# ginevracoal/robustBNNs

Measured on AMD Instinct MI355X. Metric: attack-samples/sec (test_pts x posterior_samples x PGD_iters), higher is better.
Workload: dtype f32 (full-width operands as three f16 pieces: 6 exact f16 MFMA product terms per fp32 product, f32 accumulate)

## Files before the change

include/robustbnns_hip.h:

```cpp
#ifndef ROBUSTBNNS_HIP_H
#define ROBUSTBNNS_HIP_H

#include <stddef.h>
#include <stdint.h>

#ifdef __cplusplus
extern "C" {
#endif

#define RBNN_ABI_VERSION 10
#define RBNN_CPAD 16

typedef enum rbnn_status {
    RBNN_OK = 0,
    RBNN_ERR_NULL = -1,
    RBNN_ERR_SHAPE = -2,
    RBNN_ERR_UNSUPPORTED = -3,
    RBNN_ERR_LAUNCH = -4,
    RBNN_ERR_ALIGN = -5
} rbnn_status;

typedef enum rbnn_activation { RBNN_ACT_RELU = 0, RBNN_ACT_LEAKY = 1, RBNN_ACT_SIGM = 2, RBNN_ACT_TANH = 3 } rbnn_activation;
typedef enum rbnn_arch { RBNN_ARCH_FC = 0, RBNN_ARCH_FC2 = 1 } rbnn_arch;

// ... 49 lines not shown
int rbnn_reduce_samples(const float *P, int32_t n_samples, int32_t n_points, int32_t n_classes,
                        float scale, float *out, int32_t ldo, void *stream);

int rbnn_loss_dlogits(int32_t mode, const float *P, const float *Psum, int32_t ldp, const float *G_up,
                      const int32_t *labels, int32_t n_samples, float inv_S, int32_t n_points,
                      int32_t n_classes, float *dZ, void *stream);

int rbnn_fc_input_grad(const rbnn_posterior *net, const int32_t *sample_idx, int32_t n_samples,
                       int32_t n_points, int32_t chunk, const rbnn_workspace *ws,
                       int32_t *n_slabs_out, void *stream);

int rbnn_sum_slabs(const float *slabs, int32_t n_slabs, int32_t n_points, int32_t d_pad, float scale,
                   float *out, int32_t ldo, void *stream);

int rbnn_sum_slabs_norms(const float *slabs, int32_t n_slabs, int32_t n_points, int32_t d_pad, int32_t in_features, float scale,
                         float *out, int32_t ldo, float *linf, float *l2, void *stream);

int rbnn_pgd_alpha(const float *X0, int32_t ldx, int32_t n_points, int32_t in_features,
                   float *alpha, void *stream);

int rbnn_attack_step(float *X, const float *X0, int32_t ldx, const float *G, int32_t n_slabs,
                     size_t slab_stride, int32_t ldg, const float *alpha, float alpha_scalar,
                     float eps, int32_t project, int32_t n_points, int32_t in_features, void *stream);

int rbnn_eval_metrics(const float *out_orig, const float *out_adv, int32_t ldp, const int32_t *labels,
                      int32_t n_points, int32_t n_classes, int32_t *counts, float *rob, void *stream);

int rbnn_pack_rows4(const float *W, int64_t rows, int32_t cols, float *out, void *stream);

typedef struct rbnn_dev_scale {
    uint32_t absmax_bits;
    int32_t  exp;
    float    scale;
    float    inv_scale;
} rbnn_dev_scale;

int rbnn_input_scales(const float *X, int64_t rows, int32_t cols, int32_t ld, float floor_abs, float mul, float add,
                      float cap, rbnn_dev_scale *out, void *stream);

typedef struct rbnn_conv_posterior {
    int32_t activation;
    int32_t hidden;
    int32_t n_classes;
    int32_t n_stored;
    int32_t in_channels;
    int32_t in_width;
// ... 577 lines not shown
```

robustbnns_amd/_hip.py:

```python
import ctypes as C
import os

import torch

from . import _header
from ._header import HipError

_HERE = os.path.dirname(os.path.abspath(__file__))
LIB_PATH = os.path.join(_HERE, "csrc", "librbnn_hip.so")
HEADER_PATH = os.path.join(os.path.dirname(_HERE), "include", "robustbnns_hip.h")

STRUCTS = {
    "Posterior": "rbnn_posterior", "Workspace": "rbnn_workspace", "WorkspaceSizes": "rbnn_workspace_sizes",
    "ConvPosterior": "rbnn_conv_posterior", "ConvWorkspace": "rbnn_conv_workspace", "ConvWorkspaceSizes": "rbnn_conv_workspace_sizes",
    "PieceImages": "rbnn_triple_images", "SplitImages": "rbnn_triple_images", "TripleImages": "rbnn_triple_images",
    "SplitWorkspace": "rbnn_split_workspace", "SplitWorkspaceSizes": "rbnn_split_workspace_sizes",
    "TripleWorkspace": "rbnn_triple_workspace", "TripleWorkspaceSizes": "rbnn_triple_workspace_sizes",
    "SviGuide": "rbnn_svi_guide", "SviFlatTensor": "rbnn_svi_flat_tensor", "SviTrainNet": "rbnn_svi_train_net", "SviTrainWs": "rbnn_svi_train_ws",
    "NnTrainNet": "rbnn_nn_train_net", "NnTrainWs": "rbnn_nn_train_ws",
    "ConvTrainNet": "rbnn_conv_train_net", "ConvTrainWs": "rbnn_conv_train_ws", "ConvTrainBytes": "rbnn_conv_train_bytes",
    "ConvSviTrainNet": "rbnn_conv_svi_train_net",
    "ConvEnsNet": "rbnn_conv_ens_net", "ConvEnsWs": "rbnn_conv_ens_ws", "ConvEnsBytes": "rbnn_conv_ens_bytes",
    "ConvSviLockstepNet": "rbnn_conv_svi_guides_net", "ConvSviLockstepWs": "rbnn_conv_svi_guides_ws", "ConvSviLockstepBytes": "rbnn_conv_svi_guides_bytes",
    "HmcChain": "rbnn_hmc_chain", "HmcLockstep": "rbnn_hmc_lockstep", "ConvHmcChainsNet": "rbnn_conv_hmc_chains_net", "SviLockstep": "rbnn_svi_multi", "SviLockstepAcc": "rbnn_svi_multi_acc",
# ... 120 lines not shown
        check(self.lib.rbnn_loss_dlogits(mode, ptr(P), ptr(Psum), ldp, ptr(G_up), ptr(labels), S, inv_S, N, Cn,
                                         ptr(dZ), stream_of(P)), "rbnn_loss_dlogits")

    def fc_input_grad(self, net, sidx, S, N, chunk, ws):
        w = self._ws(ws)
        n = C.c_int32(0)
        check(self.lib.rbnn_fc_input_grad(C.byref(net.descriptor()), ptr(sidx), S, N, chunk, C.byref(w), C.byref(n),
                                          stream_of(ws["dZ"])), "rbnn_fc_input_grad")
        return n.value

    def sum_slabs(self, slabs, K, N, Dp, scale, out):
        require_gpu(slabs, "slabs")
        check(self.lib.rbnn_sum_slabs(ptr(slabs), K, N, Dp, scale, ptr(out), out.stride(0), stream_of(slabs)), "rbnn_sum_slabs")

    def sum_slabs_norms(self, slabs, K, N, Dp, D, scale, out, linf, l2):
        require_gpu(slabs, "slabs")
        check(self.lib.rbnn_sum_slabs_norms(ptr(slabs), K, N, Dp, D, scale, ptr(out), out.stride(0), ptr(linf), ptr(l2),
                                            stream_of(slabs)), "rbnn_sum_slabs_norms")

    def pgd_alpha(self, X0, D, alpha):
        require_gpu(X0, "X0")
        check(self.lib.rbnn_pgd_alpha(ptr(X0), X0.stride(0), X0.shape[0], D, ptr(alpha), stream_of(X0)), "rbnn_pgd_alpha")

    def attack_step(self, X, X0, G, K, slab_stride, ldg, alpha, alpha_scalar, eps, project, D):
        require_gpu(X, "X")
        check(self.lib.rbnn_attack_step(ptr(X), ptr(X0), X.stride(0), ptr(G), K, slab_stride, ldg, ptr(alpha),
                                        alpha_scalar, eps, int(project), X.shape[0], D, stream_of(X)), "rbnn_attack_step")

    def eval_metrics(self, A, B, labels, Cn, counts, rob):
        require_gpu(A, "outputs")
        check(self.lib.rbnn_eval_metrics(ptr(A), ptr(B), A.stride(0), ptr(labels), A.shape[0], Cn, ptr(counts), ptr(rob),
                                         stream_of(A)), "rbnn_eval_metrics")

    def pack_rows4(self, W, out):
        require_gpu(W, "W")
        cols = W.shape[-1]
        check(self.lib.rbnn_pack_rows4(ptr(W), W.numel() // cols, cols, ptr(out), stream_of(W)), "rbnn_pack_rows4")

    def input_scales(self, X, cols, floor_abs, mul, add, cap, out):
        require_gpu(X, "X")
        check(self.lib.rbnn_input_scales(ptr(X), X.shape[0], cols, X.stride(0), floor_abs, mul, add, cap, ptr(out), stream_of(X)),
              "rbnn_input_scales")
        return out

    def _rows_image(self, name, src, cols, scale_exp, out, ld_dst, dev_scale):
        require_gpu(src, "src")
        ld_src = src.shape[-1]
        check(getattr(self.lib, name)(ptr(src), src.numel() // ld_src, cols, ld_src, scale_exp, ptr(dev_scale), ptr(out), ld_dst, stream_of(src)), name)
# ... 247 lines not shown
```

robustbnns_amd/csrc/rbnn_kernels.hip:

```cpp
#include "rbnn_common.hpp"
#include <stdlib.h>

namespace {

struct FwdArgs {
    const float* X;   long long x_sample_stride;  int ldx;  int N;
    const float* W;   long long w_sample_stride;  int ldw;  int KT;
    const float* b;
    const float* W2;  const float* b2;            int C;    int H;
    const int* sidx;  int S;   int NT;
    float* P;  uint32_t* mask;  float* dact;  float* hid;  int out_kind;
};

template <int ACT, int WH, int HTW, int WN, int NTW, bool LAYER2>
__global__ void __launch_bounds__(64 * WH * WN, (HTW * NTW > 16 ? 2 : (WH * WN) / 2)) fc_forward_kernel(const FwdArgs a) {
    constexpr int BH = WH * HTW * 16, BN = WN * NTW * 16;
    constexpr int TILE = (BH + BN) * 16;
    constexpr bool BITMASK = (ACT == RBNN_ACT_RELU || ACT == RBNN_ACT_LEAKY);
    constexpr int NW = WH * WN;
    static_assert(NW == 4 || NW == 8, "4 or 8 waves per block");
    static_assert(HTW % 2 == 0 && HTW <= 8, "a wave's h range is whole 32-bit mask words, at most 4");
    static_assert(WH * BN * 16 <= 2 * TILE, "the Z^T reduction scratch aliases the tile buffers");
    __shared__ __attribute__((aligned(16))) float lds[2 * TILE];
    float* const zred = lds;
// ... 468 lines not shown

__global__ void attack_step4_kernel(float* __restrict__ X, const float* __restrict__ X0, int ldx,
                                    const float* __restrict__ G, int K, long long slab_stride, int ldg,
                                    const float* __restrict__ alpha, float alpha_scalar, float eps, int project,
                                    int N, int D4) {
    const long long i = (long long)blockIdx.x * blockDim.x + threadIdx.x;
    if (i >= (long long)N * D4) return;
    const long long n = i / D4;
    const int d = 4 * (int)(i % D4);
    f32x4 g = *(const f32x4*)(G + n * ldg + d);
    for (int k = 1; k < K; ++k) g += *(const f32x4*)(G + k * slab_stride + n * ldg + d);
    const float step = alpha ? alpha[n] : alpha_scalar;
    const f32x4 x = *(const f32x4*)(X + n * ldx + d);
    f32x4 x0 = x, out;
    if (project) x0 = *(const f32x4*)(X0 + n * ldx + d);
#pragma unroll
    for (int r = 0; r < 4; ++r) {
        const float sgn = (g[r] > 0.f) ? 1.f : ((g[r] < 0.f) ? -1.f : 0.f);
        float pert = x[r] + step * sgn;
        if (project) pert = x0[r] + fminf(fmaxf(pert - x0[r], -eps), eps);
        out[r] = fminf(fmaxf(pert, 0.f), 1.f);
    }
    *(f32x4*)(X + n * ldx + d) = out;
}

__global__ void eval_metrics_kernel(const float* __restrict__ A, const float* __restrict__ B, int ldp,
                                    const int* __restrict__ labels, int N, int C, int* __restrict__ counts,
                                    float* __restrict__ rob) {
    const int n = blockIdx.x * blockDim.x + threadIdx.x;
    int ok_a = 0, ok_b = 0;
    if (n < N) {
        float ma = -INFINITY, mb = -INFINITY;
        int ia = 0, ib = 0;
        for (int c = 0; c < C; ++c) {
            const float a = A[(long long)n * ldp + c], b = B[(long long)n * ldp + c];
            if (a > ma) { ma = a; ia = c; }
            if (b > mb) { mb = b; ib = c; }
        }
        float da = 0.f, db = 0.f;
        for (int c = 0; c < C; ++c) { da += expf(A[(long long)n * ldp + c] - ma); db += expf(B[(long long)n * ldp + c] - mb); }
        float diff = 0.f;
        for (int c = 0; c < C; ++c)
            diff = fmaxf(diff, fabsf(expf(A[(long long)n * ldp + c] - ma) / da - expf(B[(long long)n * ldp + c] - mb) / db));
        rob[n] = 1.f - diff;
        ok_a = (ia == labels[n]);
        ok_b = (ib == labels[n]);
// ... 277 lines not shown
int rbnn_pgd_alpha(const float* X0, int32_t ldx, int32_t N, int32_t D, float* alpha, void* stream) {
    if (!X0 || !alpha) return RBNN_ERR_NULL;
    if (N < 1 || D < 1 || ldx < D) return RBNN_ERR_SHAPE;
    hipLaunchKernelGGL(pgd_alpha_kernel, dim3((N + 3) / 4), dim3(256), 0, (hipStream_t)stream, X0, ldx, N, D, alpha);
    return launch_status();
}

int rbnn_attack_step(float* X, const float* X0, int32_t ldx, const float* G, int32_t K, size_t slab_stride, int32_t ldg,
                     const float* alpha, float alpha_scalar, float eps, int32_t project, int32_t N, int32_t D, void* stream) {
    if (!X || !G || (project && !X0)) return RBNN_ERR_NULL;
    if (N < 1 || D < 1 || ldx < D || ldg < D || K < 1) return RBNN_ERR_SHAPE;
    if (!(D & 3) && !(ldx & 3) && !(ldg & 3) && !(slab_stride & 3) && aligned16(X) && aligned16(G) && (!project || aligned16(X0))) {
        const long long total4 = (long long)N * (D / 4);
        hipLaunchKernelGGL(attack_step4_kernel, dim3((unsigned)((total4 + 255) / 256)), dim3(256), 0, (hipStream_t)stream,
                           X, X0, ldx, G, K, (long long)slab_stride, ldg, alpha, alpha_scalar, eps, project, N, D / 4);
        return launch_status();
    }
    const long long total = (long long)N * D;
    hipLaunchKernelGGL(attack_step_kernel, dim3((unsigned)((total + 255) / 256)), dim3(256), 0, (hipStream_t)stream,
                       X, X0, ldx, G, K, (long long)slab_stride, ldg, alpha, alpha_scalar, eps, project, N, D);
    return launch_status();
}

int rbnn_eval_metrics(const float* out_orig, const float* out_adv, int32_t ldp, const int32_t* labels, int32_t N, int32_t C,
                      int32_t* counts, float* rob, void* stream) {
    if (!out_orig || !out_adv || !labels || !counts || !rob) return RBNN_ERR_NULL;
    if (N < 1 || C < 1 || ldp < C) return RBNN_ERR_SHAPE;
    if (hipMemsetAsync(counts, 0, 2 * sizeof(int32_t), (hipStream_t)stream) != hipSuccess) return RBNN_ERR_LAUNCH;
    hipLaunchKernelGGL(eval_metrics_kernel, dim3((N + 255) / 256), dim3(256), 0, (hipStream_t)stream,
                       out_orig, out_adv, ldp, labels, N, C, counts, rob);
    return launch_status();
}

int rbnn_pack_rows4(const float* W, int64_t rows, int32_t cols, float* out, void* stream) {
    if (!W || !out) return RBNN_ERR_NULL;
    if (rows < 4 || (rows & 3) || cols < 1) return RBNN_ERR_SHAPE;
    if (!aligned16(out)) return RBNN_ERR_ALIGN;
    const long long total = (rows / 4) * (long long)cols;
    hipLaunchKernelGGL(pack_rows4_kernel, dim3((unsigned)((total + 255) / 256)), dim3(256), 0, (hipStream_t)stream, W, (long long)(rows / 4), cols, out);
    return launch_status();
}

int rbnn_svi_materialize(const float* loc, const float* scale_raw, const float* eps, int64_t n_elem, int32_t S, float* out, void* stream) {
    if (!loc || !scale_raw || !eps || !out) return RBNN_ERR_NULL;
    if (n_elem < 1 || S < 1) return RBNN_ERR_SHAPE;
    const long long total = (long long)n_elem * S;
// ... 10 lines not shown
```

robustbnns_amd/csrc/rbnn_svi.hip:

```cpp
#include "rbnn_common.hpp"
#include <algorithm>

namespace {

struct DrawArgs {
    rbnn_posterior net;
    rbnn_triple_images tp;
    rbnn_svi_guide g;
    const unsigned long long* sample_keys;
    unsigned long long key;
    uint32_t draw_id;
    int S, has_tp, tiles_w1_d, tiles_wm_d, tiles_per_sample;
    int images_only;
    float w1_scale, wm_scale, w2_scale;
};

__device__ void draw_matrix_tile(const DrawArgs& a, const Rng& rng, int tensor, int s, int hb, int dt, const float* loc, const float* scl,
                                 int H0, int cols, float* W, int ldw, float* pack4, uint4* rows_img, int ld_rows, uint4* cols_img, int ld_cols,
                                 float img_scale, float (*tile)[68]) {
    const int H = a.net.hidden, t = threadIdx.x, d0 = 64 * dt;
#pragma unroll
    for (int i = 0; i < 2; ++i) {
        const int q = t + 256 * i, hl = q >> 4, dq = q & 15;
        const int h = 32 * hb + hl, c4 = (d0 >> 2) + dq;
        float w[4] = {0.f, 0.f, 0.f, 0.f};
        if (h < H0 && 4 * c4 < cols) draw_quad(rng, tensor, loc, scl, h, c4, cols, w);
        *(f32x4*)&tile[hl][4 * dq] = (f32x4){w[0], w[1], w[2], w[3]};
    }
    __syncthreads();
    if (W) {
#pragma unroll
        for (int i = 0; i < 2; ++i) {
            const int q = t + 256 * i, hl = q >> 4, dq = q & 15, d = d0 + 4 * dq;
            if (d < ldw) *(f32x4*)(W + ((long long)s * H + 32 * hb + hl) * ldw + d) = *(const f32x4*)&tile[hl][4 * dq];
        }
    }
    if (pack4) {
// ... 70 lines not shown
        const int lane = i & 63, li = lane & 15, lg = lane >> 4, k = (i >> 6) & 1, tl = i >> 7;
        _Float16 w[10][3];
#pragma unroll
        for (int c = 0; c < 10; ++c) pieces_of<3>((c < C) ? w2l[c * H + 16 * tl + li] * a.w2_scale : 0.f, w[c]);
        union { f16x8 v; uint4 u; } o;
        const _Float16 z = (_Float16)0.f;
        if (lg < 3) {
            const int piece = (k == 0) ? (lg == 2 ? 1 : 0) : (lg == 0 ? 1 : (lg == 1 ? 0 : 2));
#pragma unroll
            for (int j = 0; j < 8; ++j) o.v[j] = piece == 0 ? w[j][0] : (piece == 1 ? w[j][1] : w[j][2]);
        } else if (k == 0) {
            o.v[0] = w[8][0]; o.v[1] = w[9][0]; o.v[2] = w[8][0]; o.v[3] = w[9][0];
            o.v[4] = w[8][0]; o.v[5] = w[9][0]; o.v[6] = w[8][1]; o.v[7] = w[9][1];
        } else {
            o.v[0] = w[8][2]; o.v[1] = w[9][2]; o.v[2] = w[8][1]; o.v[3] = w[9][1];
            o.v[4] = z; o.v[5] = z; o.v[6] = z; o.v[7] = z;
        }
        gen[i] = o.u;
    }
}

__global__ void __launch_bounds__(256) svi_draw_kernel(const DrawArgs a) {
    extern __shared__ float dyn_lds[];
    const int s = blockIdx.x / a.tiles_per_sample, j = blockIdx.x % a.tiles_per_sample;
    const unsigned long long key = a.sample_keys ? a.sample_keys[s] : a.key;
    const Rng rng = {(uint32_t)key, (uint32_t)(key >> 32), a.sample_keys ? 0u : (uint32_t)s, a.draw_id};
    const int H = a.net.hidden;
    const int n_w1 = (H / 32) * a.tiles_w1_d, n_wm = (H / 32) * a.tiles_wm_d;
    float (*tile)[68] = (float (*)[68])dyn_lds;
    if (j < n_w1) {
        draw_matrix_tile(a, rng, T_W1, s, j / a.tiles_w1_d, j % a.tiles_w1_d, a.g.W1_loc, a.g.W1_scale, a.g.hidden, a.net.in_features,
                         a.images_only ? nullptr : const_cast<float*>(a.net.W1), a.net.in_stride, a.images_only ? nullptr : const_cast<float*>(a.net.W1_pack4),
                         a.has_tp ? (uint4*)const_cast<void*>(a.tp.W1_rows) : nullptr, a.tp.ld_rows,
                         a.has_tp ? (uint4*)const_cast<void*>(a.tp.W1_cols) : nullptr, a.tp.ld_cols, a.w1_scale, tile);
    } else if (j < n_w1 + n_wm) {
        const int jj = j - n_w1;
        draw_matrix_tile(a, rng, T_WM, s, jj / a.tiles_wm_d, jj % a.tiles_wm_d, a.g.Wm_loc, a.g.Wm_scale, a.g.hidden, a.g.hidden,
                         a.images_only ? nullptr : const_cast<float*>(a.net.Wm), H, a.images_only ? nullptr : const_cast<float*>(a.net.Wm_pack4),
                         a.has_tp ? (uint4*)const_cast<void*>(a.tp.Wm_rows) : nullptr, H,
                         a.has_tp ? (uint4*)const_cast<void*>(a.tp.Wm_cols) : nullptr, H, a.wm_scale, tile);
    } else {
        draw_small(a, rng, s, dyn_lds);
    }
}


struct FlatArgs {
// ... 69 lines not shown
    if (images_only && !tp) return RBNN_ERR_NULL;
    if (!g->W1_loc || !g->W1_scale || !g->b1_loc || !g->b1_scale || !g->W2_loc || !g->W2_scale || !g->b2_loc || !g->b2_scale) return RBNN_ERR_NULL;
    if (net->arch != RBNN_ARCH_FC && net->arch != RBNN_ARCH_FC2) return RBNN_ERR_UNSUPPORTED;
    const bool fc2 = net->arch == RBNN_ARCH_FC2;
    if (fc2 && (!net->Wm || !net->bm || !g->Wm_loc || !g->Wm_scale || !g->bm_loc || !g->bm_scale)) return RBNN_ERR_NULL;
    const int H = net->hidden, C = net->n_classes;
    if (n_samples < 1 || n_samples > net->n_stored || H < 32 || (H & 31) || g->hidden < 1 || g->hidden > H || C < 1 || C > 16) return RBNN_ERR_SHAPE;
    if (net->in_features < 1 || net->in_stride < net->in_features || (net->in_stride & 15)) return RBNN_ERR_SHAPE;
    DrawArgs a = {};
    a.net = *net; a.g = *g; a.sample_keys = (const unsigned long long*)sample_keys; a.key = key; a.draw_id = draw_id; a.S = n_samples;
    a.images_only = images_only;
    int extent = net->in_stride;
    if (tp) {
        if (!tp->W1_rows || !tp->W1_cols || !tp->W2_gen || (fc2 && (!tp->Wm_rows || !tp->Wm_cols))) return RBNN_ERR_NULL;
        if (tp->ld_rows < net->in_features || (tp->ld_rows & 31) || tp->ld_cols != net->in_stride || C > 10 || (H & 127)) return RBNN_ERR_SHAPE;
        if (tp->w1_exp < -100 || tp->w1_exp > 100 || tp->w2_exp < -100 || tp->w2_exp > 100 || tp->wm_exp < -100 || tp->wm_exp > 100) return RBNN_ERR_SHAPE;
        a.tp = *tp; a.has_tp = 1;
        a.w1_scale = ldexpf(1.f, tp->w1_exp); a.w2_scale = ldexpf(1.f, tp->w2_exp); a.wm_scale = ldexpf(1.f, tp->wm_exp);
        extent = std::max(extent, (int)tp->ld_rows);
    }
    a.tiles_w1_d = (extent + 63) / 64;
    a.tiles_wm_d = fc2 ? (H + 63) / 64 : 0;
    a.tiles_per_sample = (H / 32) * (a.tiles_w1_d + a.tiles_wm_d) + 1;
    const size_t lds = std::max((size_t)32 * 68 * sizeof(float), (size_t)C * H * sizeof(float));
    if (lds > SVI_DRAW_LDS_MAX) return RBNN_ERR_SHAPE;
    static unsigned long long attr = 0;
    if (lds > 64 * 1024 && !ensure_dynamic_lds((const void*)svi_draw_kernel, (int)SVI_DRAW_LDS_MAX, attr)) return RBNN_ERR_LAUNCH;
    hipLaunchKernelGGL(svi_draw_kernel, dim3((unsigned)((long long)n_samples * a.tiles_per_sample)), dim3(256), lds, (hipStream_t)stream, a);
    return launch_status();
}

int rbnn_svi_draw(const rbnn_posterior* net, const rbnn_triple_images* tp, const rbnn_svi_guide* g, int32_t n_samples,
                  const uint64_t* sample_keys, uint64_t key, uint32_t draw_id, void* stream) {
    return svi_draw_impl(net, tp, g, n_samples, sample_keys, key, draw_id, 0, stream);
}

int rbnn_svi_draw_images(const rbnn_posterior* net, const rbnn_triple_images* tp, const rbnn_svi_guide* g, int32_t n_samples,
                         const uint64_t* sample_keys, uint64_t key, uint32_t draw_id, void* stream) {
    return svi_draw_impl(net, tp, g, n_samples, sample_keys, key, draw_id, 1, stream);
}

}

#include "rbnn_svi_step.hpp"
#include "rbnn_conv_layout.hpp"

// ... 34 lines not shown
```

robustbnns_amd/csrc/rbnn_triple.hip:

```cpp
#include "rbnn_pieces.hpp"
#include <algorithm>
#include <cstdlib>

namespace {

#ifndef RBNN_X3_PAIR_NOP
#define RBNN_X3_PAIR_NOP 0
#endif
#if RBNN_X3_PAIR_NOP
#define RBNN_X3_PAIR_PAD "\n\ts_nop 1"
#else
#define RBNN_X3_PAIR_PAD ""
#endif
#define RBNN_X3_PAIR_BODY \
    "v_bfe_i32 %[me], %[mw], %[b0], 1\n\t" \
    "v_bfe_i32 %[mo], %[mw], %[b1], 1\n\t" \
    "v_bfi_b32 %[me], %[me], %[cp], %[cn]\n\t" \
    "v_bfi_b32 %[mo], %[mo], %[cp], %[cn]\n\t" \
    "v_fma_mixlo_f16 %[d0], %[ge], %[me], 0\n\t" \
    "v_fma_mixhi_f16 %[d0], %[go], %[mo], 0\n\t" \
    "v_fma_mix_f32 %[re], %[ge], %[me], -%[d0] op_sel_hi:[0,0,1]\n\t" \
    "v_fma_mix_f32 %[ro], %[go], %[mo], -%[d0] op_sel:[0,0,1] op_sel_hi:[0,0,1]\n\t" \
    "v_cvt_pk_f16_f32 %[d1], %[re], %[ro]\n\t" \
    "v_fma_mixlo_f16 %[d2], -%[d1], %[one], %[re] op_sel_hi:[1,0,0]\n\t" \
// ... 605 lines not shown
    for (int s = q; s < S; s += 16) {
        _Float16 d[10][3];
        float dz[16];
#pragma unroll
        for (int c = 0; c < 16; ++c) dz[c] = 0.f;
        if (n < N) tail_dz<MODE>(P + ((long long)s * N + n) * RBNN_CPAD, gmean, y, C, inv_S, dz);
#pragma unroll
        for (int c = 0; c < 10; ++c) pieces_of<3>((n < N && c < C) ? ldexpf(dz[c], e) : 0.f, d[c]);
        uint4* const o = dst + ((long long)s * N_pad + n) * 4;
#pragma unroll
        for (int ch = 0; ch < 3; ++ch) {
            union { f16x8 v; uint4 u; } w;
#pragma unroll
            for (int j = 0; j < 8; ++j) w.v[j] = d[j][ch];
            o[ch ^ sw] = w.u;
        }
        union { f16x8 v; uint4 u; } t;
        t.v[0] = d[8][0]; t.v[1] = d[9][0]; t.v[2] = d[8][1]; t.v[3] = d[9][1];
        t.v[4] = d[8][2]; t.v[5] = d[9][2]; t.v[6] = d[8][0]; t.v[7] = d[9][0];
        o[3 ^ sw] = t.u;
    }
}

__global__ void __launch_bounds__(256) attack_step_x3_kernel(float* __restrict__ X, const float* __restrict__ X0, int ldx, const float* __restrict__ G,
                                                             int K, long long slab_stride, int ldg, const float* __restrict__ alpha, float alpha_scalar,
                                                             float eps, int project, long long N, int D, const rbnn_dev_scale* __restrict__ ds,
                                                             uint4* __restrict__ dst, int groups) {
    const long long i = (long long)blockIdx.x * blockDim.x + threadIdx.x;
    if (i >= N * groups) return;
    const long long n = i / groups;
    const int gq = (int)(i % groups), d0 = 8 * gq;
    const float scale = ds->scale;
    float xn[8];
#pragma unroll
    for (int j = 0; j < 8; ++j) xn[j] = 0.f;
    if (d0 < D) {
        const float step = alpha ? alpha[n] : alpha_scalar;
#pragma unroll
        for (int h = 0; h < 2; ++h) {
            const int d = d0 + 4 * h;
            if (d < D) {
                f32x4 g = *(const f32x4*)(G + n * ldg + d);
                for (int k = 1; k < K; ++k) g += *(const f32x4*)(G + k * slab_stride + n * ldg + d);
                const f32x4 x = *(const f32x4*)(X + n * ldx + d);
                f32x4 x0 = x, out;
                if (project) x0 = *(const f32x4*)(X0 + n * ldx + d);
// ... 289 lines not shown
    }
    return ok[dev] == 1;
}

template <int ACT, int MODE>
int launch_grad_x3(const GradPieceArgs& a, hipStream_t st) {
    if constexpr (MODE == GRAD_FC && (ACT == RBNN_ACT_RELU || ACT == RBNN_ACT_LEAKY)) {
        if (x3_grad_td9() && (a.Dt + 8) / 9 < (a.Dt + 6) / 7 && x3_grad_two_blocks<ACT, 9, MODE>()) return launch_grad_x3_cfg<ACT, 9, MODE>(a, st);
    }
    if constexpr (MODE != GRAD_FC2_STEP2 && (ACT == RBNN_ACT_RELU || ACT == RBNN_ACT_LEAKY)) {
        if (x3_grad_td9() && (a.Dt + 7) / 8 < (a.Dt + 6) / 7 && x3_grad_two_blocks<ACT, 8, MODE>()) return launch_grad_x3_cfg<ACT, 8, MODE>(a, st);
    }
    if ((a.Dt + 6) / 7 < (a.Dt + 3) / 4) return launch_grad_x3_cfg<ACT, 7, MODE>(a, st);
    return launch_grad_x3_cfg<ACT, 4, MODE>(a, st);
}

template <int MODE>
int launch_grad_x3_act(int act, const GradPieceArgs& a, hipStream_t st) {
    return for_activation(act, [&](auto A) {
        return launch_grad_x3<(decltype(A)::value == RBNN_ACT_TANH ? RBNN_ACT_SIGM : decltype(A)::value), MODE>(a, st);
    });
}

}

extern "C" {

int rbnn_triple_rows(const float* src, int64_t rows, int32_t cols, int32_t ld_src, int32_t scale_exp,
                     const rbnn_dev_scale* dev_scale, void* dst, int32_t ld_dst, void* stream) {
    return launch_rows_image(triple_rows_kernel, src, rows, cols, ld_src, scale_exp, dev_scale, dst, ld_dst, stream, 0);
}

int rbnn_triple_rows_grouped(const float* src, int64_t rows, int32_t cols, int32_t ld_src, int32_t scale_exp,
                             const rbnn_dev_scale* dev_scale, void* dst, int32_t ld_dst, void* stream) {
    return launch_rows_image(triple_rows_kernel, src, rows, cols, ld_src, scale_exp, dev_scale, dst, ld_dst, stream, 1);
}

int rbnn_triple_cols(const float* W, int64_t n_mats, int32_t rows, int32_t cols, int32_t ld_src, int32_t scale_exp,
                     void* dst, int32_t ld_dst, void* stream) {
    return launch_cols_image(triple_cols_kernel, W, n_mats, rows, cols, ld_src, scale_exp, dst, ld_dst, stream);
}

int rbnn_triple_w2gen(const float* W2, int32_t n_mats, int32_t C, int32_t H, int32_t scale_exp, void* dst, void* stream) {
    return launch_w2gen_image(triple_w2gen_kernel, 128, W2, n_mats, C, H, scale_exp, dst, stream);
}

// ... 13 lines not shown
int rbnn_fc_forward_triple(const rbnn_posterior* net, const rbnn_triple_images* tp, const rbnn_triple_workspace* tws,
                           int32_t x_exp, const rbnn_dev_scale* dev_scales, int32_t N, const int32_t* sidx, int32_t S,
                           int32_t out_kind, const rbnn_workspace* ws, void* stream) {
    FwdX3Args a = {}, b = {};
    int rc = fc_forward_pieces_args(net, tp, tws ? tws->X_triple : nullptr, tp ? tp->ld_rows : 0, tws ? tws->hid_triple : nullptr, 6, 15,
                                    x_exp, dev_scales, N, sidx, S, out_kind, ws, a, b);
    if (rc) return rc;
    hipStream_t st = (hipStream_t)stream;
    a.x_group_bytes = (unsigned)a.KT * 3072u; a.x_stage_bytes = 3072u;
    if (net->arch != RBNN_ARCH_FC2) return launch_forward_x3<true>(net->activation, a, st);
    if ((rc = launch_forward_x3<false>(net->activation, a, st))) return rc;
    const int NG = (N + 15) / 16;
    b.x_sample_bytes = (long long)NG * 16 * net->hidden * 4; b.x_group_bytes = 2048u; b.x_stage_bytes = (unsigned)NG * 2048u;
    return launch_forward_x3<true, true>(net->activation, b, st);
}

int rbnn_step_tail_triple(int32_t mode, const float* P, const int32_t* labels, int32_t S, float inv_S, int32_t N, int32_t C, float* Psum_out,
                          int32_t ldo, const rbnn_triple_workspace* tws, void* stream) {
    if (!P || !labels || !tws || !tws->dZ_gen || !tws->g_scale) return RBNN_ERR_NULL;
    if (mode != RBNN_LOSS_MEAN_PROB && mode != RBNN_LOSS_PER_SAMPLE && mode != RBNN_LOSS_MEAN_LOGIT) return RBNN_ERR_UNSUPPORTED;
    if (S < 1 || N < 1 || C < 1 || C > 10 || (Psum_out && ldo < C)) return RBNN_ERR_SHAPE;
    if (!aligned16(P) || !aligned16(tws->dZ_gen)) return RBNN_ERR_ALIGN;
    const long long n_pad = mask_ld(N);
    const dim3 grid((unsigned)(n_pad / 16)), block(256);
    hipStream_t st = (hipStream_t)stream;
    if (mode == RBNN_LOSS_MEAN_PROB)
        hipLaunchKernelGGL(step_tail_x3_kernel<RBNN_LOSS_MEAN_PROB>, grid, block, 0, st, P, labels, S, inv_S, N, n_pad, C, Psum_out, ldo, (uint4*)tws->dZ_gen, tws->g_scale);
    else if (mode == RBNN_LOSS_PER_SAMPLE)
        hipLaunchKernelGGL(step_tail_x3_kernel<RBNN_LOSS_PER_SAMPLE>, grid, block, 0, st, P, labels, S, inv_S, N, n_pad, C, Psum_out, ldo, (uint4*)tws->dZ_gen, tws->g_scale);
    else
        hipLaunchKernelGGL(step_tail_x3_kernel<RBNN_LOSS_MEAN_LOGIT>, grid, block, 0, st, P, labels, S, inv_S, N, n_pad, C, Psum_out, ldo, (uint4*)tws->dZ_gen, tws->g_scale);
    return launch_status();
}

int rbnn_attack_step_triple(float* X, const float* X0, int32_t ldx, const float* G, int32_t K, size_t slab_stride, int32_t ldg, const float* alpha,
                            float alpha_scalar, float eps, int32_t project, int32_t N, int32_t D, const rbnn_dev_scale* dev_scale, void* X_triple,
                            int32_t ld_rows, void* stream) {
    if (!X || !G || (project && !X0) || !dev_scale || !X_triple) return RBNN_ERR_NULL;
    if (N < 1 || D < 1 || ldx < D || ldg < D || K < 1 || ld_rows < D || (ld_rows & 31)) return RBNN_ERR_SHAPE;
    if ((D & 3) || (ldx & 3) || (ldg & 3) || (slab_stride & 3)) return RBNN_ERR_SHAPE;
    if (!aligned16(X) || !aligned16(G) || (project && !aligned16(X0)) || !aligned16(X_triple)) return RBNN_ERR_ALIGN;
    const int groups = ld_rows / 8;
    const long long total = (long long)N * groups;
    hipLaunchKernelGGL(attack_step_x3_kernel, dim3((unsigned)((total + 255) / 256)), dim3(256), 0, (hipStream_t)stream,
                       X, X0, ldx, G, K, (long long)slab_stride, ldg, alpha, alpha_scalar, eps, project, (long long)N, D, dev_scale, (uint4*)X_triple, groups);
    return launch_status();
}

// ... 11 lines not shown
```

robustbnns_amd/engine.py:

```python
import os

import torch

from . import _hip
from ._hip import (LOSS_MEAN_LOGIT, LOSS_MEAN_PROB, LOSS_PER_SAMPLE, LOSS_UPSTREAM, LOSS_UPSTREAM_LOGIT, OUT_LOGITS, OUT_PROBS)
from .fp64_core import Fp64Core, wgrad_arguments
from .posterior import LAYER_KEYS

_WS_DTYPE = {"mask1": torch.int32, "mask2": torch.int32}


def to_labels(y, device):
    y = torch.as_tensor(y)
    if y.dim() >= 2:
        y = y.argmax(-1)
    return y.to(device=device, dtype=torch.int32).contiguous()


class _DifferentiableForward(torch.autograd.Function):

    @staticmethod
    def forward(ctx, x, engine, sidx, S, logits):
        ctx.engine, ctx.sidx, ctx.S, ctx.logits = engine, sidx, S, logits
        ctx.save_for_backward(x.detach())
# ... 416 lines not shown
        for k, shp in shapes.items():
            if fc2 or k not in ("dWm", "dbm"):
                n = S * int(torch.Size(shp).numel())
                out[k] = self.fp64.buffer(-(-n // 2) * 16)[:n].view((S,) + shp).zero_()
        ce = self.fp64.buffer(-(-S * N // 2) * 16)[:S * N].view(S, N)
        blocks = self.fp64.point_blocks(N, S, 2)
        G = self.fp64.buffer((blocks[0][1] - blocks[0][0]) * p.Dp * 8).view(-1, p.Dp)
        for lo, hi in blocks:
            n = hi - lo
            ws = {**self.fp64.workspace(n, S), **self.fp64.workspace(n, S, 1)}
            self.k.fc_forward_f64(p, X[lo:hi], sidx, S, OUT_LOGITS, ws)
            self.k.conv_head_ce_dp(ws["P"], labels[lo:hi], S, n, p.C, 1.0 / N if reduction == "mean" else 1.0, ws["dZ"], ws["ce"])
            self.k.fc_hidden_dp(p, X[lo:hi], sidx, S, ws)
            self.k.fc_input_grad_f64(p, sidx, S, n, ws, 1.0, G[:n])
            self.k.fc_weight_grads_dp(p, X[lo:hi], S, ws, out)
            ce[:, lo:hi] = ws["ce"].view(S, n)
        if p.Hp != p.H:
            real = {"dW1": (p.H, p.D), "db1": (p.H,), "dWm": (p.H, p.H), "dbm": (p.H,), "dW2": (p.C, p.H), "db2": (p.C,)}
            out = {k: v[(slice(None),) + tuple(slice(0, d) for d in real[k])].contiguous() for k, v in out.items()}
        names = [k for k in _hip.FC_WGRAD_DP_OUT_KEYS if k in out]
        keys = [layer + sfx for layer in LAYER_KEYS[p.arch] for sfx in (".weight", ".bias")]
        return dict(zip(keys, (out[k] for k in names))), ce

    def _step(self, X, X0, labels, sidx, S, mode, alpha, alpha_scalar, eps, project):
        p = self.post
        if self.precision == "fp64":
            return self.fp64.step(X, X0, labels, sidx, S, mode, alpha, alpha_scalar, eps, project)
        if self.world > 1 and self.pipelined_comm:
            return self._step_sharded(X, X0, labels, sidx, S, mode, alpha, alpha_scalar, eps, project)
        ws, n_slabs, _ = self.gradient_slabs(X, labels, sidx, S, mode)
        if (self.world == 1 and self._carry_image and self._fused_tail(mode, None) and self._scales is not None and "triple" in ws
                and p.D % 4 == 0):
            self.k.attack_step_triple(X, X0, ws["slabs"], n_slabs, X.shape[0] * p.Dp, p.Dp, alpha, alpha_scalar, eps, project, p.D,
                                      self._scales, ws["triple"]["X_triple"], self.post.triple_images().ld_rows)
            ws["x_image_ready"] = X.data_ptr()
        elif self.world == 1:
            self.k.attack_step(X, X0, ws["slabs"], n_slabs, X.shape[0] * p.Dp, p.Dp, alpha, alpha_scalar, eps, project, p.D)
        else:
            G = ws["Gsum"] if "Gsum" in ws else ws["G"]
            self.k.sum_slabs(ws["slabs"], n_slabs, X.shape[0], p.Dp, 1.0, G)
            self._allreduce(G)
            self.k.attack_step(X, X0, G, 1, 0, p.Dp, alpha, alpha_scalar, eps, project, p.D)

    pipelined_comm = True

    def _comm_blocks(self, N, S=None):
        env = os.environ.get("RBNN_COMM_BLOCKS")
        if env is not None:
            want = int(env)
        else:
            want = 2 if (S is not None and S * getattr(self.post, "Hp", 1 << 30) < 16384) else 1
        return max(1, min(want, N // max(1, int(os.environ.get("RBNN_COMM_MIN_POINTS", "512")))))

    def _step_sharded(self, X, X0, labels, sidx, S, mode, alpha, alpha_scalar, eps, project):
        p, N, C = self.post, X.shape[0], self.post.C
        nb = self._comm_blocks(N, S)
        bounds = [0] + [min(N, (N * i // nb + 255) // 256 * 256) for i in range(1, nb)] + [N]
        bounds = sorted(set(bounds))
# ... 9 lines not shown
            h = None
            if need_psum:
                self.k.reduce_samples(ws["P"], S, hi - lo, C, 1.0, ws["Psum"])
                h = self._allreduce_async(ws["Psum"])
            blocks.append((lo, hi, ws, h))
        pending = []
        for lo, hi, ws, h in blocks:
            if h is not None:
                self._wait(h)
            self.k.loss_dlogits(mode, ws["P"], ws["Psum"] if need_psum else None, None, labels[lo:hi], S, inv_S, hi - lo, C, ws["dZ"])
            n_slabs = self._grad_kernels(sidx, S, hi - lo, ws)
            self.k.sum_slabs(ws["slabs"], n_slabs, hi - lo, p.Dp, 1.0, ws["G"])
            pending.append(self._allreduce_async(ws["G"]))
        for (lo, hi, ws, _), h in zip(blocks, pending):
            self._wait(h)
            self.k.attack_step(X[lo:hi], None if X0 is None else X0[lo:hi], ws["G"], 1, 0, p.Dp,
                               None if alpha is None else alpha[lo:hi], alpha_scalar, eps, project, p.D)

    def fgsm(self, x, y, n_samples, epsilon=0.3, seeds=None, mode=LOSS_MEAN_PROB):
        sidx, S = self.sample_index(n_samples, seeds)
        if self.precision == "lowdim":
            out = self._lowdim_attack(self._flat(x), None, to_labels(y, self.device), sidx, S, mode, None, 0.0, False, float(epsilon), False, 1)
            return out.reshape(x.shape)
        X = self.pad_inputs(x, clone=True)
        self._scales = self._input_scales(X, iterates=False)
        try:
            self._step(X, None, to_labels(y, self.device), sidx, S, mode, None, float(epsilon), 0.0, False)
        finally:
            self._scales = None
        return self.unpad(X, x)

    def attack_gradient(self, x, y, n_samples, seeds=None, mode=LOSS_MEAN_PROB):
        sidx, S = self.sample_index(n_samples, seeds)
        xin = self._flat(x) if self.precision == "lowdim" else self.pad_inputs(x)
        return self.gradient(xin, to_labels(y, self.device), sidx, S, mode).clone()

    def fgsm_from_gradient(self, x, G, epsilon):
        p = self.post
        X = self.pad_inputs(x, clone=True)
        if G.dtype == torch.float64:
            self.k.attack_step_f64(X, None, G, None, float(epsilon), 0.0, False, p.D)
            return self.unpad(X, x)
        self.k.attack_step(X, None, G, 1, 0, p.Dp, None, float(epsilon), 0.0, False, p.D)
        return self.unpad(X, x)

    shared_forward = True

    def loss_gradients_and_fgsm(self, x, y, n_samples, epsilon=0.3, seeds=None, mode=LOSS_MEAN_PROB):
        if not self.shared_forward or self.precision in ("lowdim", "fp64") or mode != LOSS_MEAN_PROB:
            return self.loss_gradients(x, y, n_samples, seeds), self.fgsm(x, y, n_samples, epsilon, seeds, mode)
        sidx, S = self.sample_index(n_samples, seeds)
        labels = to_labels(y, self.device)
        p = self.post
        X = self.pad_inputs(x, clone=True)
        N = X.shape[0]
        self._scales = self._input_scales(X, iterates=False)
        try:
            ws = self.workspace(N, S)
            S_tot = self.total_samples(S)
            self._forward_kernels(X, sidx, S, OUT_PROBS, ws)
            G = ws["Gsum"] if "Gsum" in ws else ws["G"]
# ... 155 lines not shown
```

Measured before the change: 142.7 million.

## Add out-of-place attack step, LDS-staged triple tail kernel, and SVI draw order option

Adds an out-of-place attack step kernel so FGSM paths write into a fresh buffer instead of cloning the padded input first. It also adds a staged step-tail kernel for the triple-precision path that loads the per-sample probabilities into LDS once and reuses them for the sum, max-scale and dz passes. This staged kernel is on by default, with a budget-based points-per-block choice. An env-gated sample-fastest block ordering is added for the SVI draw kernel. The changes are mostly independent and add extra code paths plus more LDS use per block.

```diff
diff --git a/include/robustbnns_hip.h b/include/robustbnns_hip.h
--- a/include/robustbnns_hip.h
+++ b/include/robustbnns_hip.h
@@ -95,6 +95,10 @@
 int rbnn_attack_step(float *X, const float *X0, int32_t ldx, const float *G, int32_t n_slabs,
                      size_t slab_stride, int32_t ldg, const float *alpha, float alpha_scalar,
                      float eps, int32_t project, int32_t n_points, int32_t in_features, void *stream);
+
+int rbnn_attack_step_out(const float *Xin, float *Xout, const float *X0, int32_t ldx, const float *G, int32_t n_slabs,
+                         size_t slab_stride, int32_t ldg, const float *alpha, float alpha_scalar,
+                         float eps, int32_t project, int32_t n_points, int32_t in_features, void *stream);
 
 int rbnn_eval_metrics(const float *out_orig, const float *out_adv, int32_t ldp, const int32_t *labels,
                       int32_t n_points, int32_t n_classes, int32_t *counts, float *rob, void *stream);
diff --git a/robustbnns_amd/_hip.py b/robustbnns_amd/_hip.py
--- a/robustbnns_amd/_hip.py
+++ b/robustbnns_amd/_hip.py
@@ -166,8 +166,15 @@
         require_gpu(X0, "X0")
         check(self.lib.rbnn_pgd_alpha(ptr(X0), X0.stride(0), X0.shape[0], D, ptr(alpha), stream_of(X0)), "rbnn_pgd_alpha")
 
-    def attack_step(self, X, X0, G, K, slab_stride, ldg, alpha, alpha_scalar, eps, project, D):
-        require_gpu(X, "X")
+    def attack_step(self, X, X0, G, K, slab_stride, ldg, alpha, alpha_scalar, eps, project, D, out=None):
+        require_gpu(X, "X")
+        if out is not None:
+            require_gpu(out, "out")
+            if out.shape != X.shape or out.stride(0) != X.stride(0):
+                raise HipError(f"out {tuple(out.shape)} (row stride {out.stride(0)}) must have X's shape {tuple(X.shape)} and row stride {X.stride(0)}")
+            check(self.lib.rbnn_attack_step_out(ptr(X), ptr(out), ptr(X0), X.stride(0), ptr(G), K, slab_stride, ldg, ptr(alpha),
+                                                alpha_scalar, eps, int(project), X.shape[0], D, stream_of(X)), "rbnn_attack_step_out")
+            return
         check(self.lib.rbnn_attack_step(ptr(X), ptr(X0), X.stride(0), ptr(G), K, slab_stride, ldg, ptr(alpha),
                                         alpha_scalar, eps, int(project), X.shape[0], D, stream_of(X)), "rbnn_attack_step")
 
diff --git a/robustbnns_amd/csrc/rbnn_kernels.hip b/robustbnns_amd/csrc/rbnn_kernels.hip
--- a/robustbnns_amd/csrc/rbnn_kernels.hip
+++ b/robustbnns_amd/csrc/rbnn_kernels.hip
@@ -514,6 +514,52 @@
         out[r] = fminf(fmaxf(pert, 0.f), 1.f);
     }
     *(f32x4*)(X + n * ldx + d) = out;
+}
+
+__global__ void attack_step_out_kernel(const float* Xin, float* Xout, const float* __restrict__ X0, int ldx,
+                                       const float* __restrict__ G, int K, long long slab_stride, int ldg,
+                                       const float* __restrict__ alpha, float alpha_scalar, float eps, int project,
+                                       int N, int D) {
+    const long long i = (long long)blockIdx.x * blockDim.x + threadIdx.x;
+    if (i >= (long long)N * D) return;
+    const long long n = i / D;
+    const int d = (int)(i % D);
+    float g = G[n * ldg + d];
+    for (int k = 1; k < K; ++k) g += G[k * slab_stride + n * ldg + d];
+    const float sgn = (g > 0.f) ? 1.f : ((g < 0.f) ? -1.f : 0.f);
+    const float step = alpha ? alpha[n] : alpha_scalar;
+    const float x = Xin[n * ldx + d];
+    float pert = x + step * sgn;
+    if (project) {
+        const float x0 = X0[n * ldx + d];
+        const float eta = fminf(fmaxf(pert - x0, -eps), eps);
+        pert = x0 + eta;
+    }
+    Xout[n * ldx + d] = fminf(fmaxf(pert, 0.f), 1.f);
+}
+
+__global__ void attack_step4_out_kernel(const float* Xin, float* Xout, const float* __restrict__ X0, int ldx,
+                                        const float* __restrict__ G, int K, long long slab_stride, int ldg,
+                                        const float* __restrict__ alpha, float alpha_scalar, float eps, int project,
+                                        int N, int D4) {
+    const long long i = (long long)blockIdx.x * blockDim.x + threadIdx.x;
+    if (i >= (long long)N * D4) return;
+    const long long n = i / D4;
+    const int d = 4 * (int)(i % D4);
+    f32x4 g = *(const f32x4*)(G + n * ldg + d);
+    for (int k = 1; k < K; ++k) g += *(const f32x4*)(G + k * slab_stride + n * ldg + d);
+    const float step = alpha ? alpha[n] : alpha_scalar;
+    const f32x4 x = *(const f32x4*)(Xin + n * ldx + d);
+    f32x4 x0 = x, out;
+    if (project) x0 = *(const f32x4*)(X0 + n * ldx + d);
+#pragma unroll
+    for (int r = 0; r < 4; ++r) {
+        const float sgn = (g[r] > 0.f) ? 1.f : ((g[r] < 0.f) ? -1.f : 0.f);
+        float pert = x[r] + step * sgn;
+        if (project) pert = x0[r] + fminf(fmaxf(pert - x0[r], -eps), eps);
+        out[r] = fminf(fmaxf(pert, 0.f), 1.f);
+    }
+    *(f32x4*)(Xout + n * ldx + d) = out;
 }
 
 __global__ void eval_metrics_kernel(const float* __restrict__ A, const float* __restrict__ B, int ldp,
@@ -837,6 +883,22 @@
     return launch_status();
 }
 
+int rbnn_attack_step_out(const float* Xin, float* Xout, const float* X0, int32_t ldx, const float* G, int32_t K, size_t slab_stride, int32_t ldg,
+                         const float* alpha, float alpha_scalar, float eps, int32_t project, int32_t N, int32_t D, void* stream) {
+    if (!Xin || !Xout || !G || (project && !X0)) return RBNN_ERR_NULL;
+    if (N < 1 || D < 1 || ldx < D || ldg < D || K < 1) return RBNN_ERR_SHAPE;
+    if (!(D & 3) && !(ldx & 3) && !(ldg & 3) && !(slab_stride & 3) && aligned16(Xin) && aligned16(Xout) && aligned16(G) && (!project || aligned16(X0))) {
+        const long long total4 = (long long)N * (D / 4);
+        hipLaunchKernelGGL(attack_step4_out_kernel, dim3((unsigned)((total4 + 255) / 256)), dim3(256), 0, (hipStream_t)stream,
+                           Xin, Xout, X0, ldx, G, K, (long long)slab_stride, ldg, alpha, alpha_scalar, eps, project, N, D / 4);
+        return launch_status();
+    }
+    const long long total = (long long)N * D;
+    hipLaunchKernelGGL(attack_step_out_kernel, dim3((unsigned)((total + 255) / 256)), dim3(256), 0, (hipStream_t)stream,
+                       Xin, Xout, X0, ldx, G, K, (long long)slab_stride, ldg, alpha, alpha_scalar, eps, project, N, D);
+    return launch_status();
+}
+
 int rbnn_eval_metrics(const float* out_orig, const float* out_adv, int32_t ldp, const int32_t* labels, int32_t N, int32_t C,
                       int32_t* counts, float* rob, void* stream) {
     if (!out_orig || !out_adv || !labels || !counts || !rob) return RBNN_ERR_NULL;
diff --git a/robustbnns_amd/csrc/rbnn_svi.hip b/robustbnns_amd/csrc/rbnn_svi.hip
--- a/robustbnns_amd/csrc/rbnn_svi.hip
+++ b/robustbnns_amd/csrc/rbnn_svi.hip
@@ -1,5 +1,6 @@
 #include "rbnn_common.hpp"
 #include <algorithm>
+#include <cstdlib>
 
 namespace {
 
@@ -13,6 +14,7 @@
     int S, has_tp, tiles_w1_d, tiles_wm_d, tiles_per_sample;
     int images_only;
     float w1_scale, wm_scale, w2_scale;
+    int sample_fastest;
 };
 
 __device__ void draw_matrix_tile(const DrawArgs& a, const Rng& rng, int tensor, int s, int hb, int dt, const float* loc, const float* scl,
@@ -129,7 +131,8 @@
 
 __global__ void __launch_bounds__(256) svi_draw_kernel(const DrawArgs a) {
     extern __shared__ float dyn_lds[];
-    const int s = blockIdx.x / a.tiles_per_sample, j = blockIdx.x % a.tiles_per_sample;
+    const int s = a.sample_fastest ? blockIdx.x % a.S : blockIdx.x / a.tiles_per_sample;
+    const int j = a.sample_fastest ? blockIdx.x / a.S : blockIdx.x % a.tiles_per_sample;
     const unsigned long long key = a.sample_keys ? a.sample_keys[s] : a.key;
     const Rng rng = {(uint32_t)key, (uint32_t)(key >> 32), a.sample_keys ? 0u : (uint32_t)s, a.draw_id};
     const int H = a.net.hidden;
@@ -245,6 +248,10 @@
     a.tiles_w1_d = (extent + 63) / 64;
     a.tiles_wm_d = fc2 ? (H + 63) / 64 : 0;
     a.tiles_per_sample = (H / 32) * (a.tiles_w1_d + a.tiles_wm_d) + 1;
+    {
+        const char* const e = getenv("RBNN_SVI_DRAW_ORDER");
+        a.sample_fastest = e && e[0] != '0' && e[0] != '\0';
+    }
     const size_t lds = std::max((size_t)32 * 68 * sizeof(float), (size_t)C * H * sizeof(float));
     if (lds > SVI_DRAW_LDS_MAX) return RBNN_ERR_SHAPE;
     static unsigned long long attr = 0;
diff --git a/robustbnns_amd/csrc/rbnn_triple.hip b/robustbnns_amd/csrc/rbnn_triple.hip
--- a/robustbnns_amd/csrc/rbnn_triple.hip
+++ b/robustbnns_amd/csrc/rbnn_triple.hip
@@ -651,6 +651,92 @@
     }
 }
 
+template <int MODE, int PB>
+__global__ void __launch_bounds__(256) step_tail_x3_staged_kernel(const float* __restrict__ P, const int* __restrict__ labels, int S, float inv_S, int N,
+                                                                  long long N_pad, int C, float* __restrict__ Psum_out, int ldo,
+                                                                  uint4* __restrict__ dst, float* __restrict__ gscale) {
+    constexpr int Q = 256 / PB;
+    extern __shared__ __attribute__((aligned(16))) float lds[];
+    __shared__ float red[Q][PB + 1];
+    __shared__ float psum[PB][16];
+    const int p = threadIdx.x % PB, q = threadIdx.x / PB;
+    const long long n0 = (long long)blockIdx.x * PB, n = n0 + p;
+    {
+        const int rows = (int)min((long long)PB, (long long)N - n0);
+#pragma unroll 4
+        for (int i = threadIdx.x; i < S * PB * 4; i += 256) {
+            const int s = i / (PB * 4), c = i % (PB * 4);
+            f32x4 v = (f32x4){0.f, 0.f, 0.f, 0.f};
+            if ((c >> 2) < rows) v = *(const f32x4*)(P + ((long long)s * N + n0) * RBNN_CPAD + 4 * c);
+            *(f32x4*)(lds + 4 * i) = v;
+        }
+    }
+    __syncthreads();
+    if (MODE != RBNN_LOSS_PER_SAMPLE) {
+        if (q < 4) {
+            f32x4 sum = (f32x4){0.f, 0.f, 0.f, 0.f};
+            if (n < N)
+#pragma unroll 8
+                for (int s = 0; s < S; ++s) sum += *(const f32x4*)(lds + (s * PB + p) * RBNN_CPAD + 4 * q);
+#pragma unroll
+            for (int r = 0; r < 4; ++r) {
+                psum[p][4 * q + r] = sum[r];
+                if (Psum_out && n < N && 4 * q + r < C) Psum_out[n * ldo + 4 * q + r] = sum[r];
+            }
+        }
+        __syncthreads();
+    }
+    const int y = (n < N) ? labels[n] : 0;
+    float gmean[16];
+    if (MODE != RBNN_LOSS_PER_SAMPLE) {
+        float t[16];
+#pragma unroll
+        for (int c = 0; c < 16; ++c) t[c] = (c < C) ? psum[p][c] * inv_S : 0.f;
+        ce_softmax_grad<16>(t, C, y, inv_S, gmean);
+    } else {
+#pragma unroll
+        for (int c = 0; c < 16; ++c) gmean[c] = 0.f;
+    }
+    float m = 0.f;
+    if (n < N)
+        for (int s = q; s < S; s += Q) {
+            float dz[16];
+            tail_dz<MODE>(lds + (s * PB + p) * RBNN_CPAD, gmean, y, C, inv_S, dz);
+#pragma unroll
+            for (int c = 0; c < 12; ++c) if (c < C) m = fmaxf(m, fabsf(dz[c]));
+        }
+    red[q][p] = m;
+    __syncthreads();
+    m = 0.f;
+#pragma unroll
+    for (int i = 0; i < Q; ++i) m = fmaxf(m, red[i][p]);
+    int e = 0;
+    if (m > 0.f && m < INFINITY) e = min(13 - ilogbf(m), 120);
+    if (q == 0) gscale[n] = ldexpf(1.f, -e);
+    const int sw = dz_swz3(n);
+    for (int s = q; s < S; s += Q) {
+        _Float16 d[10][3];
+        float dz[16];
+#pragma unroll
+        for (int c = 0; c < 16; ++c) dz[c] = 0.f;
+        if (n < N) tail_dz<MODE>(lds + (s * PB + p) * RBNN_CPAD, gmean, y, C, inv_S, dz);
+#pragma unroll
+        for (int c = 0; c < 10; ++c) pieces_of<3>((n < N && c < C) ? ldexpf(dz[c], e) : 0.f, d[c]);
+        uint4* const o = dst + ((long long)s * N_pad + n) * 4;
+#pragma unroll
+        for (int ch = 0; ch < 3; ++ch) {
+            union { f16x8 v; uint4 u; } w;
+#pragma unroll
+            for (int j = 0; j < 8; ++j) w.v[j] = d[j][ch];
+            o[ch ^ sw] = w.u;
+        }
+        union { f16x8 v; uint4 u; } t;
+        t.v[0] = d[8][0]; t.v[1] = d[9][0]; t.v[2] = d[8][1]; t.v[3] = d[9][1];
+        t.v[4] = d[8][2]; t.v[5] = d[9][2]; t.v[6] = d[8][0]; t.v[7] = d[9][0];
+        o[3 ^ sw] = t.u;
+    }
+}
+
 __global__ void __launch_bounds__(256) attack_step_x3_kernel(float* __restrict__ X, const float* __restrict__ X0, int ldx, const float* __restrict__ G,
                                                              int K, long long slab_stride, int ldg, const float* __restrict__ alpha, float alpha_scalar,
                                                              float eps, int project, long long N, int D, const rbnn_dev_scale* __restrict__ ds,
@@ -986,6 +1072,39 @@
     });
 }
 
+constexpr long long TAIL_STAGE_BUDGET = 32 * 1024, TAIL_STAGE_MAX = 128 * 1024;
+
+inline long long tail_stage_budget() {
+    const char* const e = getenv("RBNN_TAIL_STAGE_KB");
+    const long kb = e ? strtol(e, nullptr, 10) : 0;
+    return (kb >= 1 && kb <= TAIL_STAGE_MAX / 1024) ? kb * 1024 : TAIL_STAGE_BUDGET;
+}
+
+struct TailArgs {
+    const float* P; const int* labels; int S; float inv_S; int N; long long n_pad; int C; float* Psum_out; int ldo; uint4* dst; float* gscale;
+};
+
+template <int MODE, int PB>
+int launch_tail_staged_cfg(const TailArgs& t, hipStream_t st) {
+    auto kern = step_tail_x3_staged_kernel<MODE, PB>;
+    const int ldsb = t.S * PB * 64;
+    static unsigned long long attr_done = 0;
+    if (!ensure_dynamic_lds((const void*)kern, (int)TAIL_STAGE_MAX, attr_done)) return RBNN_ERR_LAUNCH;
+    hipLaunchKernelGGL(kern, dim3((unsigned)(t.n_pad / PB)), dim3(256), ldsb, st, t.P, t.labels, t.S, t.inv_S, t.N, t.n_pad, t.C, t.Psum_out, t.ldo,
+                       t.dst, t.gscale);
+    return launch_status();
+}
+
+template <int MODE>
+int launch_tail_staged(int PB, const TailArgs& t, hipStream_t st) {
+    switch (PB) {
+        case 16: return launch_tail_staged_cfg<MODE, 16>(t, st);
+        case 8: return launch_tail_staged_cfg<MODE, 8>(t, st);
+        case 4: return launch_tail_staged_cfg<MODE, 4>(t, st);
+        default: return launch_tail_staged_cfg<MODE, 2>(t, st);
+    }
+}
+
 }
 
 extern "C" {
@@ -1045,8 +1164,17 @@
     if (S < 1 || N < 1 || C < 1 || C > 10 || (Psum_out && ldo < C)) return RBNN_ERR_SHAPE;
     if (!aligned16(P) || !aligned16(tws->dZ_gen)) return RBNN_ERR_ALIGN;
     const long long n_pad = mask_ld(N);
+    hipStream_t st = (hipStream_t)stream;
+    const char* const sw = getenv("RBNN_TAIL_STAGED");
+    if ((!sw || sw[0] != '0') && (long long)S * 2 * 64 <= TAIL_STAGE_MAX) {
+        const long long budget = tail_stage_budget();
+        const int PB = (long long)S * 16 * 64 <= budget ? 16 : (long long)S * 8 * 64 <= budget ? 8 : (long long)S * 4 * 64 <= budget ? 4 : 2;
+        const TailArgs t = {P, labels, S, inv_S, N, n_pad, C, Psum_out, ldo, (uint4*)tws->dZ_gen, tws->g_scale};
+        if (mode == RBNN_LOSS_MEAN_PROB) return launch_tail_staged<RBNN_LOSS_MEAN_PROB>(PB, t, st);
+        if (mode == RBNN_LOSS_PER_SAMPLE) return launch_tail_staged<RBNN_LOSS_PER_SAMPLE>(PB, t, st);
+        return launch_tail_staged<RBNN_LOSS_MEAN_LOGIT>(PB, t, st);
+    }
     const dim3 grid((unsigned)(n_pad / 16)), block(256);
-    hipStream_t st = (hipStream_t)stream;
     if (mode == RBNN_LOSS_MEAN_PROB)
         hipLaunchKernelGGL(step_tail_x3_kernel<RBNN_LOSS_MEAN_PROB>, grid, block, 0, st, P, labels, S, inv_S, N, n_pad, C, Psum_out, ldo, (uint4*)tws->dZ_gen, tws->g_scale);
     else if (mode == RBNN_LOSS_PER_SAMPLE)
diff --git a/robustbnns_amd/engine.py b/robustbnns_amd/engine.py
--- a/robustbnns_amd/engine.py
+++ b/robustbnns_amd/engine.py
@@ -462,7 +462,10 @@
         keys = [layer + sfx for layer in LAYER_KEYS[p.arch] for sfx in (".weight", ".bias")]
         return dict(zip(keys, (out[k] for k in names))), ce
 
-    def _step(self, X, X0, labels, sidx, S, mode, alpha, alpha_scalar, eps, project):
+    def _step_out_of_place(self):
+        return isinstance(self.k, _hip.HipKernels) and self.post.Dp == self.post.D and os.environ.get("RBNN_STEP_OUT") != "0"
+
+    def _step(self, X, X0, labels, sidx, S, mode, alpha, alpha_scalar, eps, project, out=None):
         p = self.post
         if self.precision == "fp64":
             return self.fp64.step(X, X0, labels, sidx, S, mode, alpha, alpha_scalar, eps, project)
@@ -474,6 +477,8 @@
             self.k.attack_step_triple(X, X0, ws["slabs"], n_slabs, X.shape[0] * p.Dp, p.Dp, alpha, alpha_scalar, eps, project, p.D,
                                       self._scales, ws["triple"]["X_triple"], self.post.triple_images().ld_rows)
             ws["x_image_ready"] = X.data_ptr()
+        elif self.world == 1 and out is not None:
+            self.k.attack_step(X, X0, ws["slabs"], n_slabs, X.shape[0] * p.Dp, p.Dp, alpha, alpha_scalar, eps, project, p.D, out=out)
         elif self.world == 1:
             self.k.attack_step(X, X0, ws["slabs"], n_slabs, X.shape[0] * p.Dp, p.Dp, alpha, alpha_scalar, eps, project, p.D)
         else:
@@ -529,13 +534,15 @@
         if self.precision == "lowdim":
             out = self._lowdim_attack(self._flat(x), None, to_labels(y, self.device), sidx, S, mode, None, 0.0, False, float(epsilon), False, 1)
             return out.reshape(x.shape)
-        X = self.pad_inputs(x, clone=True)
+        out_of_place = self.world == 1 and self.precision != "fp64" and self._step_out_of_place()
+        X = self.pad_inputs(x, clone=not out_of_place)
+        out = torch.empty_like(X) if out_of_place else None
         self._scales = self._input_scales(X, iterates=False)
         try:
-            self._step(X, None, to_labels(y, self.device), sidx, S, mode, None, float(epsilon), 0.0, False)
+            self._step(X, None, to_labels(y, self.device), sidx, S, mode, None, float(epsilon), 0.0, False, out=out)
         finally:
             self._scales = None
-        return self.unpad(X, x)
+        return out.reshape(x.shape) if out_of_place else self.unpad(X, x)
 
     def attack_gradient(self, x, y, n_samples, seeds=None, mode=LOSS_MEAN_PROB):
         sidx, S = self.sample_index(n_samples, seeds)
@@ -544,6 +551,11 @@
 
     def fgsm_from_gradient(self, x, G, epsilon):
         p = self.post
+        if G.dtype != torch.float64 and self._step_out_of_place():
+            X = self.pad_inputs(x)
+            out = torch.empty_like(X)
+            self.k.attack_step(X, None, G, 1, 0, p.Dp, None, float(epsilon), 0.0, False, p.D, out=out)
+            return out.reshape(x.shape)
         X = self.pad_inputs(x, clone=True)
         if G.dtype == torch.float64:
             self.k.attack_step_f64(X, None, G, None, float(epsilon), 0.0, False, p.D)
```

Result: no change. 143.1 million, median of 3 (+0.3%).
